# Litianyu141/Gen-FVGN-steady

Hardware: AMD Instinct MI355X
Metric: training iters/sec, 50k-cell cylinder mesh (fwd + loss + bwd + Adam, batch resident in HBM) (higher is better)
Workload: dtype f32

## Files before the change

gen-fvgn-steady_amd/csrc/slice.hip:

```cpp
#include <cstdlib>
#include "gfv_common.h"
#include "gfv_prof.h"
#include "../../include/gfv.h"

namespace {

constexpr int H = 8, D = 16, G = 32;

__global__ __launch_bounds__(256) void slice_softmax_fwd_kernel(const float* __restrict__ xmid, const float* __restrict__ Ws,
                                                                const float* __restrict__ bs, const float* __restrict__ temp,
                                                                float* __restrict__ w, int N) {
  __shared__ float sW[G * D];
  __shared__ float sB[G];
  __shared__ __attribute__((aligned(16))) float stage[256 * (G + 4)];
  const int tid = threadIdx.x;
  for (int i = tid; i < G * D; i += 256) sW[i] = Ws[i];
  if (tid < G) sB[tid] = bs[tid];
  __syncthreads();
  const long row0 = (long)blockIdx.x * 256;
  const long row = row0 + tid;
  const long nrows = (long)N * H;
  if (row < nrows) {
    const int h = (int)(row & (H - 1));
    float x[D];
// ... 304 lines not shown
    for (int c = 0; c < D; ++c) {
      const float t = sTok[g][c];
      q += t * sWq[j * D + c]; k += t * sWk[j * D + c]; v += t * sWv[j * D + c];
    }
    sQ[g][j] = q; sK[g][j] = k; sV[g][j] = v;
  }
  __syncthreads();
  for (int idx = tid; idx < G * D; idx += 256) {
    const int j = idx / D, c = idx % D;
    float s = 0.f;
    for (int i = 0; i < G; ++i) s += sA[i][j] * sGO[i][c];
    sGV[j][c] = s;
  }
  for (int idx = tid; idx < G * G; idx += 256) {
    const int i = idx / G, j = idx % G;
    float s = 0.f;
#pragma unroll
    for (int c = 0; c < D; ++c) s += sGO[i][c] * sV[j][c];
    sGA[i][j] = s;
  }
  __syncthreads();
  if (tid < G) {
    float dot = 0.f;
    for (int j = 0; j < G; ++j) dot += sA[tid][j] * sGA[tid][j];
    for (int j = 0; j < G; ++j) sGA[tid][j] = sA[tid][j] * (sGA[tid][j] - dot) * A.scale;
  }
  __syncthreads();
  for (int idx = tid; idx < G * D; idx += 256) {
    const int i = idx / D, c = idx % D;
    float gq = 0.f, gk = 0.f;
    for (int j = 0; j < G; ++j) {
      gq += sGA[i][j] * sK[j][c];
      gk += sGA[j][i] * sQ[j][c];
    }
    sGQ[i][c] = gq; sGK[i][c] = gk;
  }
  __syncthreads();
  for (int idx = tid; idx < G * D; idx += 256) {
    const int g = idx / D, c = idx % D;
    float s = 0.f;
#pragma unroll
    for (int j = 0; j < D; ++j) s += sGQ[g][j] * sWq[j * D + c] + sGK[g][j] * sWk[j * D + c] + sGV[g][j] * sWv[j * D + c];
    sGT[g][c] = s;
  }
  {
    const int j = tid / D, c = tid % D;
    float dq = 0.f, dk = 0.f, dv = 0.f;
    for (int g = 0; g < G; ++g) {
      const float t = sTok[g][c];
      dq += sGQ[g][j] * t; dk += sGK[g][j] * t; dv += sGV[g][j] * t;
    }
    float* o = A.dW_partial + (size_t)bh * 3 * D * D;
    o[tid] = dq; o[D * D + tid] = dk; o[2 * D * D + tid] = dv;
  }
  __syncthreads();
  for (int idx = tid; idx < G * D; idx += 256) {
    const int g = idx / D, c = idx % D;
    A.g_raw[(size_t)bh * G * D + idx] = sGT[g][c] / (A.norm[bh * G + g] + 1e-5f);
  }
  if (tid < G) {
    float s = 0.f;
#pragma unroll
    for (int c = 0; c < D; ++c) s += sGT[tid][c] * sTok[tid][c];
    A.g_norm[bh * G + tid] = -s / (A.norm[bh * G + tid] + 1e-5f);
  }
}

constexpr int TS = G * D + 4;

__device__ __forceinline__ bool stage_T(const float* __restrict__ T, const int* __restrict__ batch, int N, float* sT) {
  const int n_first = blockIdx.x * 32;
  const int n_last = min(n_first + 31, N - 1);
  const int b0 = batch[n_first];
  const bool uniform = (batch[n_last] == b0);
  if (uniform) {
    const float4* src = reinterpret_cast<const float4*>(T + (size_t)b0 * H * G * D);
    for (int i = threadIdx.x; i < H * G * D / 4; i += 256) {
      const int h = i / (G * D / 4), r = i % (G * D / 4);
      *reinterpret_cast<float4*>(&sT[h * TS + 4 * r]) = src[i];
    }
  }
  __syncthreads();
  return uniform;
}

__device__ __forceinline__ void deslice_row(const float4* __restrict__ wp, const float* __restrict__ Tp, float (&acc)[D]) {
#pragma unroll
  for (int i = 0; i < 8; ++i) {
    const float4 wv = wp[i];
    const float ww[4] = {wv.x, wv.y, wv.z, wv.w};
#pragma unroll
    for (int k = 0; k < 4; ++k) {
      const float4* tp = reinterpret_cast<const float4*>(Tp + (4 * i + k) * D);
#pragma unroll
      for (int j = 0; j < 4; ++j) {
        const float4 t = tp[j];
        acc[4 * j] += ww[k] * t.x; acc[4 * j + 1] += ww[k] * t.y; acc[4 * j + 2] += ww[k] * t.z; acc[4 * j + 3] += ww[k] * t.w;
      }
    }
  }
}

__global__ __launch_bounds__(256) void deslice_kernel(const float* __restrict__ w, const float* __restrict__ T,
                                                      const int* __restrict__ batch, float* __restrict__ out, int N,
                                                      int accumulate) {
  __shared__ __attribute__((aligned(16))) float sT[H * TS];
  if (accumulate & 2) {
    const int n_first = blockIdx.x * 32;
    if (batch[min(n_first + 31, N - 1)] == batch[n_first]) return;
    accumulate = 0;
  }
  const bool uniform = stage_T(T, batch, N, sT);
  const long row = (long)blockIdx.x * 256 + threadIdx.x;
  if (row >= (long)N * H) return;
  const int n = (int)(row >> 3), h = (int)(row & 7);
  float acc[D];
#pragma unroll
  for (int c = 0; c < D; ++c) acc[c] = 0.f;
  const float4* wp = reinterpret_cast<const float4*>(w + row * G);
  if (uniform) deslice_row(wp, &sT[h * TS], acc);
  else deslice_row(wp, T + ((size_t)batch[n] * H + h) * G * D, acc);
  float4* op = reinterpret_cast<float4*>(out + row * D);
#pragma unroll
  for (int j = 0; j < 4; ++j) {
    float4 v = make_float4(acc[4 * j], acc[4 * j + 1], acc[4 * j + 2], acc[4 * j + 3]);
    if (accumulate) { const float4 p = op[j]; v.x += p.x; v.y += p.y; v.z += p.z; v.w += p.w; }
    op[j] = v;
  }
}

__global__ __launch_bounds__(256) void slice_gw_kernel(const float* __restrict__ a, const float* __restrict__ T,
                                                       const float* __restrict__ add, const int* __restrict__ batch,
                                                       float* __restrict__ gw, int N, int accumulate) {
  __shared__ __attribute__((aligned(16))) float sT[H * TS];
  constexpr int SS = G + 4;
  __shared__ __attribute__((aligned(16))) float stage[256 * SS];
  const bool uniform = stage_T(T, batch, N, sT);
  const int tid = threadIdx.x;
  const long row0 = (long)blockIdx.x * 256;
  const long row = row0 + tid;
  const long nrows = (long)N * H;
  if (row < nrows) {
    const int n = (int)(row >> 3), h = (int)(row & 7);
    const size_t bh = (size_t)batch[n] * H + h;
    float x[D];
    const float4* ap = reinterpret_cast<const float4*>(a + row * D);
#pragma unroll
    for (int i = 0; i < 4; ++i) {
      const float4 v = ap[i];
      x[4 * i] = v.x; x[4 * i + 1] = v.y; x[4 * i + 2] = v.z; x[4 * i + 3] = v.w;
    }
    float4 av[G / 4];
#pragma unroll
    for (int i = 0; i < G / 4; ++i)
      av[i] = add ? reinterpret_cast<const float4*>(add + bh * G)[i] : make_float4(0.f, 0.f, 0.f, 0.f);
    const float* Tp = uniform ? &sT[h * TS] : T + bh * G * D;
#pragma unroll
    for (int i = 0; i < G / 4; ++i) {
      float r[4] = {av[i].x, av[i].y, av[i].z, av[i].w};
#pragma unroll
      for (int k = 0; k < 4; ++k) {
        const float4* tp = reinterpret_cast<const float4*>(Tp + (4 * i + k) * D);
#pragma unroll
        for (int j = 0; j < 4; ++j) {
          const float4 t = tp[j];
          r[k] += x[4 * j] * t.x + x[4 * j + 1] * t.y + x[4 * j + 2] * t.z + x[4 * j + 3] * t.w;
// ... 100 lines not shown
          const float4 t = t2[j];
          r2[k] += fx[4 * j] * t.x + fx[4 * j + 1] * t.y + fx[4 * j + 2] * t.z + fx[4 * j + 3] * t.w;
          acc[4 * j] += wg * t.x; acc[4 * j + 1] += wg * t.y; acc[4 * j + 2] += wg * t.z; acc[4 * j + 3] += wg * t.w;
        }
        gv[4 * i + k] = r2[k] + r1[k];
      }
      __builtin_amdgcn_sched_barrier(0);
    }
    float4* op = reinterpret_cast<float4*>(A.gfxmid + row * D);
#pragma unroll
    for (int j = 0; j < 4; ++j) op[j] = make_float4(acc[4 * j], acc[4 * j + 1], acc[4 * j + 2], acc[4 * j + 3]);
  }
  __syncthreads();
  if (live) {
    float x[D];
    const float4* xp = reinterpret_cast<const float4*>(A.xmid + row * D);
#pragma unroll
    for (int i = 0; i < 4; ++i) {
      const float4 v = xp[i];
      x[4 * i] = v.x; x[4 * i + 1] = v.y; x[4 * i + 2] = v.z; x[4 * i + 3] = v.w;
    }
    float dot = 0.f;
#pragma unroll
    for (int i = 0; i < 8; ++i)
      dot += wv[4 * i] * gv[4 * i] + wv[4 * i + 1] * gv[4 * i + 1] + wv[4 * i + 2] * gv[4 * i + 2] + wv[4 * i + 3] * gv[4 * i + 3];
    float gx[D];
#pragma unroll
    for (int c = 0; c < D; ++c) gx[c] = 0.f;
#pragma unroll
    for (int g = 0; g < G; ++g) {
      const float gz = wv[g] * (gv[g] - dot);
      float lg = 0.f;
#pragma unroll
      for (int c = 0; c < D; ++c) lg += x[c] * sW[g * D + c];
      lg += sB[g];
      dT -= gz * lg * invT * invT;
      const float gl = gz * invT;
      sGL[tid * (G + 1) + g] = gl;
#pragma unroll
      for (int c = 0; c < D; ++c) gx[c] += gl * sW[g * D + c];
    }
    float4* op = reinterpret_cast<float4*>(A.gxmid + row * D);
#pragma unroll
    for (int i = 0; i < 4; ++i) op[i] = make_float4(gx[4 * i], gx[4 * i + 1], gx[4 * i + 2], gx[4 * i + 3]);
#pragma unroll
    for (int c = 0; c < D; ++c) sX[tid * (D + 1) + c] = x[c];
  } else {
#pragma unroll
    for (int g = 0; g < G; ++g) sGL[tid * (G + 1) + g] = 0.f;
#pragma unroll
    for (int c = 0; c < D; ++c) sX[tid * (D + 1) + c] = 0.f;
  }
  __syncthreads();
  sDT[tid] = dT;
  __syncthreads();
  float* out = A.partial + (size_t)blockIdx.x * 552;
  {
    const int wave = tid >> 6, lane = tid & 63, li = lane & 15, kq = lane >> 4;
    if (wave < 2) {
      floatx4 acc = {0.f, 0.f, 0.f, 0.f};
#pragma unroll 8
      for (int ks = 0; ks < 64; ++ks) {
        const int r = 4 * ks + kq;
        const float a = sGL[r * (G + 1) + 16 * wave + li];
        const float b = sX[r * (D + 1) + li];
        acc = __builtin_amdgcn_mfma_f32_16x16x4f32(a, b, acc, 0, 0, 0);
      }
#pragma unroll
      for (int reg = 0; reg < 4; ++reg) out[(16 * wave + 4 * kq + reg) * D + li] = acc[reg];
    }
  }
  if (tid < G) {
    float s = 0.f;
    for (int r = 0; r < 256; ++r) s += sGL[r * (G + 1) + tid];
    out[512 + tid] = s;
  }
  if (tid < H) {
    float s = 0.f;
    for (int r = tid; r < 256; r += H) s += sDT[r];
    out[544 + tid] = s;
  }
}

__global__ __launch_bounds__(256, 2) void slice_post_bwd_mfma_kernel(const SlicePostArgs A) {
  __shared__ __attribute__((aligned(16))) float sT1[H * TS];
  __shared__ __attribute__((aligned(16))) float sT2[H * TS];
  __shared__ __attribute__((aligned(16))) float sWs[G * D];
  __shared__ float sBs[G];
  constexpr int TRS = G + 4;
  __shared__ __attribute__((aligned(16))) float sTr[4][16 * TRS];
  __shared__ float sRed[4][552];
  const int tid = threadIdx.x, wave = tid >> 6, lane = tid & 63, li = lane & 15, q = lane >> 4;
  const int n_first = blockIdx.x * 32;
  const int n_last = min(n_first + 31, A.N - 1);
  const int b0 = A.batch[n_first];
  if (A.batch[n_last] != b0) return;
  {
    const float4* s1 = reinterpret_cast<const float4*>(A.T1 + (size_t)b0 * H * G * D);
    const float4* s2 = reinterpret_cast<const float4*>(A.T2 + (size_t)b0 * H * G * D);
    for (int i = tid; i < H * G * D / 4; i += 256) {
      const int h = i / (G * D / 4), r = i % (G * D / 4);
      *reinterpret_cast<float4*>(&sT1[h * TS + 4 * r]) = s1[i];
      *reinterpret_cast<float4*>(&sT2[h * TS + 4 * r]) = s2[i];
    }
    for (int i = tid; i < G * D; i += 256) sWs[i] = A.Ws[i];
    if (tid < G) sBs[tid] = A.bs[tid];
  }
  __syncthreads();
  float bws[2][4], wsd[2][4], bsv[2];
#pragma unroll
  for (int t = 0; t < 2; ++t) {
    const float4 v = *reinterpret_cast<const float4*>(&sWs[(16 * t + li) * D + 4 * q]);
    bws[t][0] = v.x; bws[t][1] = v.y; bws[t][2] = v.z; bws[t][3] = v.w;
    bsv[t] = sBs[16 * t + li];
#pragma unroll
    for (int s = 0; s < 4; ++s) wsd[t][s] = sWs[(16 * t + 4 * q + s) * D + li];
  }
  floatx4 dws[2] = {{0.f, 0.f, 0.f, 0.f}, {0.f, 0.f, 0.f, 0.f}};
  float dbs[2] = {0.f, 0.f}, dTw[2] = {0.f, 0.f};
  float* tr = sTr[wave];
#pragma unroll 1
  for (int hh = 0; hh < 2; ++hh) {
    const int h = 2 * wave + hh;
    const float invT = 1.0f / A.temp[h];
    float b1[2][4], b2[2][4], t2d[2][4], gnv[2];
#pragma unroll
    for (int t = 0; t < 2; ++t) {
      const float4 u1 = *reinterpret_cast<const float4*>(&sT1[h * TS + (16 * t + li) * D + 4 * q]);
      const float4 u2 = *reinterpret_cast<const float4*>(&sT2[h * TS + (16 * t + li) * D + 4 * q]);
      b1[t][0] = u1.x; b1[t][1] = u1.y; b1[t][2] = u1.z; b1[t][3] = u1.w;
      b2[t][0] = u2.x; b2[t][1] = u2.y; b2[t][2] = u2.z; b2[t][3] = u2.w;
      gnv[t] = A.gnorm[((size_t)b0 * H + h) * G + 16 * t + li];
#pragma unroll
      for (int s = 0; s < 4; ++s) t2d[t][s] = sT2[h * TS + (16 * t + 4 * q + s) * D + li];
    }
#pragma unroll 1
    for (int nt = 0; nt < 2; ++nt) {
      const int n0 = n_first + 16 * nt;
      const int nodeA = n0 + li;
      const bool liveA = nodeA < A.N;
      const size_t rowA = (size_t)(liveA ? nodeA : A.N - 1) * H + h;
      const float mA = liveA ? 1.0f : 0.0f;
      float4 vgo = *reinterpret_cast<const float4*>(A.gox + rowA * D + 4 * q);
      float4 vfx = *reinterpret_cast<const float4*>(A.fxm + rowA * D + 4 * q);
      float4 vx = *reinterpret_cast<const float4*>(A.xmid + rowA * D + 4 * q);
      float4 vw0 = *reinterpret_cast<const float4*>(A.w + rowA * G + 4 * q);
      float4 vw1 = *reinterpret_cast<const float4*>(A.w + rowA * G + 16 + 4 * q);
      const float ago[4] = {vgo.x * mA, vgo.y * mA, vgo.z * mA, vgo.w * mA};
      const float afx[4] = {vfx.x * mA, vfx.y * mA, vfx.z * mA, vfx.w * mA};
      const float ax[4] = {vx.x * mA, vx.y * mA, vx.z * mA, vx.w * mA};
      const float aw[2][4] = {{vw0.x * mA, vw0.y * mA, vw0.z * mA, vw0.w * mA}, {vw1.x * mA, vw1.y * mA, vw1.z * mA, vw1.w * mA}};
      float wd[2][4], xb[4];
      size_t rowD[4];
      bool liveD[4];
#pragma unroll
      for (int r = 0; r < 4; ++r) {
        const int nd = n0 + 4 * q + r;
        liveD[r] = nd < A.N;
        rowD[r] = (size_t)(liveD[r] ? nd : A.N - 1) * H + h;
        const float m = liveD[r] ? 1.0f : 0.0f;
        wd[0][r] = A.w[rowD[r] * G + li] * m;
        wd[1][r] = A.w[rowD[r] * G + 16 + li] * m;
        xb[r] = A.xmid[rowD[r] * D + li] * m;
      }
      floatx4 g2[2], g1[2], lg[2];
#pragma unroll
      for (int t = 0; t < 2; ++t) {
        g2[t] = floatx4{gnv[t], gnv[t], gnv[t], gnv[t]};
        g1[t] = floatx4{0.f, 0.f, 0.f, 0.f};
        lg[t] = floatx4{bsv[t], bsv[t], bsv[t], bsv[t]};
#pragma unroll
        for (int s = 0; s < 4; ++s) {
          g2[t] = __builtin_amdgcn_mfma_f32_16x16x4f32(afx[s], b2[t][s], g2[t], 0, 0, 0);
          g1[t] = __builtin_amdgcn_mfma_f32_16x16x4f32(ago[s], b1[t][s], g1[t], 0, 0, 0);
          lg[t] = __builtin_amdgcn_mfma_f32_16x16x4f32(ax[s], bws[t][s], lg[t], 0, 0, 0);
        }
      }
      float gl[2][4];
#pragma unroll
      for (int r = 0; r < 4; ++r) {
        const float gw0 = g2[0][r] + g1[0][r], gw1 = g2[1][r] + g1[1][r];
        const float dot = gfv_row16_sum(wd[0][r] * gw0 + wd[1][r] * gw1);
        const float gz0 = wd[0][r] * (gw0 - dot), gz1 = wd[1][r] * (gw1 - dot);
        dTw[hh] -= (gz0 * lg[0][r] + gz1 * lg[1][r]) * invT * invT;
        gl[0][r] = gz0 * invT;
        gl[1][r] = gz1 * invT;
      }
#pragma unroll
      for (int t = 0; t < 2; ++t) {
#pragma unroll
        for (int s = 0; s < 4; ++s) dws[t] = __builtin_amdgcn_mfma_f32_16x16x4f32(gl[t][s], xb[s], dws[t], 0, 0, 0);
        dbs[t] += (gl[t][0] + gl[t][1]) + (gl[t][2] + gl[t][3]);
#pragma unroll
        for (int r = 0; r < 4; ++r) tr[(4 * q + r) * TRS + 16 * t + li] = gl[t][r];
      }
      __builtin_amdgcn_wave_barrier();
      floatx4 gxa = {0.f, 0.f, 0.f, 0.f}, gfa = {0.f, 0.f, 0.f, 0.f};
#pragma unroll
      for (int u = 0; u < 2; ++u) {
        const float4 v = *reinterpret_cast<const float4*>(&tr[li * TRS + 16 * u + 4 * q]);
        const float agl[4] = {v.x, v.y, v.z, v.w};
#pragma unroll
        for (int s = 0; s < 4; ++s) {
          gxa = __builtin_amdgcn_mfma_f32_16x16x4f32(agl[s], wsd[u][s], gxa, 0, 0, 0);
          gfa = __builtin_amdgcn_mfma_f32_16x16x4f32(aw[u][s], t2d[u][s], gfa, 0, 0, 0);
        }
      }
      __builtin_amdgcn_wave_barrier();
#pragma unroll
      for (int r = 0; r < 4; ++r) {
        if (liveD[r]) {
          A.gxmid[rowD[r] * D + li] = gxa[r];
          A.gfxmid[rowD[r] * D + li] = gfa[r];
        }
      }
    }
  }
  float* red = sRed[wave];
#pragma unroll
  for (int t = 0; t < 2; ++t) {
#pragma unroll
    for (int r = 0; r < 4; ++r) red[(16 * t + 4 * q + r) * D + li] = dws[t][r];
    float a, b;
    gfv_lane_xor16(dbs[t], a, b);
    const float v = a + b;
    gfv_lane_xor32(v, a, b);
    if (q == 0) red[512 + 16 * t + li] = a + b;
  }
#pragma unroll
  for (int hh = 0; hh < 2; ++hh) {
    const float v = gfv_wave_sum(dTw[hh]);
    if (lane == 0) red[544 + hh] = v;
  }
  __syncthreads();
  float* out = A.partial + (size_t)blockIdx.x * 552;
  for (int i = tid; i < 544; i += 256) out[i] = (sRed[0][i] + sRed[1][i]) + (sRed[2][i] + sRed[3][i]);
  if (tid < H) out[544 + tid] = sRed[tid >> 1][544 + (tid & 1)];
}

template <bool SOFTMAX>
__global__ __launch_bounds__(256, 2) void slice_token_mfma_kernel(const float* __restrict__ xmid, const float* __restrict__ Ws,
                                                                  const float* __restrict__ bs, const float* __restrict__ temp,
                                                                  float* __restrict__ w, const float* __restrict__ a,
                                                                  const int* __restrict__ chunk_beg, const int* __restrict__ chunk_end,
                                                                  float* __restrict__ partial) {
  const int tid = threadIdx.x, wave = tid >> 6, lane = tid & 63, li = lane & 15, q = lane >> 4;
  const int beg = chunk_beg[blockIdx.x], end = chunk_end[blockIdx.x];
  float bws[2][4], bsv[2];
  if (SOFTMAX) {
#pragma unroll
    for (int t = 0; t < 2; ++t) {
      const float4 v = *reinterpret_cast<const float4*>(Ws + (16 * t + li) * D + 4 * q);
      bws[t][0] = v.x; bws[t][1] = v.y; bws[t][2] = v.z; bws[t][3] = v.w;
      bsv[t] = bs[16 * t + li];
    }
  }
  float* out = partial + (size_t)blockIdx.x * 256 * 17;
#pragma unroll 1
  for (int hh = 0; hh < 2; ++hh) {
    const int h = 2 * wave + hh;
    const float invT = SOFTMAX ? 1.0f / temp[h] : 0.f;
    floatx4 tok[2] = {{0.f, 0.f, 0.f, 0.f}, {0.f, 0.f, 0.f, 0.f}};
    float nrm[2] = {0.f, 0.f};
#pragma unroll 1
    for (int n0 = beg; n0 < end; n0 += 16) {
      float wd[2][4], ab[4];
      size_t rowD[4];
      bool liveD[4];
#pragma unroll
      for (int r = 0; r < 4; ++r) {
        const int nd = n0 + 4 * q + r;
        liveD[r] = nd < end;
        rowD[r] = (size_t)(liveD[r] ? nd : end - 1) * H + h;
        ab[r] = liveD[r] ? a[rowD[r] * D + li] : 0.f;
      }
      if (SOFTMAX) {
        const int nA = n0 + li;
        const bool liveA = nA < end;
        const size_t rowA = (size_t)(liveA ? nA : end - 1) * H + h;
        const float4 vx = *reinterpret_cast<const float4*>(xmid + rowA * D + 4 * q);
        const float ax[4] = {vx.x, vx.y, vx.z, vx.w};
        floatx4 lg[2];
#pragma unroll
        for (int t = 0; t < 2; ++t) {
          lg[t] = floatx4{bsv[t], bsv[t], bsv[t], bsv[t]};
#pragma unroll
          for (int s = 0; s < 4; ++s) lg[t] = __builtin_amdgcn_mfma_f32_16x16x4f32(ax[s], bws[t][s], lg[t], 0, 0, 0);
        }
#pragma unroll
        for (int r = 0; r < 4; ++r) {
          const float z0 = lg[0][r] * invT, z1 = lg[1][r] * invT;
          const float mx = gfv_row16_max(fmaxf(z0, z1));
          const float e0 = __expf(z0 - mx), e1 = __expf(z1 - mx);
          const float inv = 1.0f / gfv_row16_sum(e0 + e1);
          const float m = liveD[r] ? 1.0f : 0.0f;
          wd[0][r] = e0 * inv * m;
          wd[1][r] = e1 * inv * m;
          if (liveD[r]) {
            w[rowD[r] * G + li] = wd[0][r];
            w[rowD[r] * G + 16 + li] = wd[1][r];
          }
        }
      } else {
#pragma unroll
        for (int r = 0; r < 4; ++r) {
          wd[0][r] = liveD[r] ? w[rowD[r] * G + li] : 0.f;
          wd[1][r] = liveD[r] ? w[rowD[r] * G + 16 + li] : 0.f;
        }
      }
#pragma unroll
      for (int t = 0; t < 2; ++t) {
#pragma unroll
        for (int s = 0; s < 4; ++s) tok[t] = __builtin_amdgcn_mfma_f32_16x16x4f32(wd[t][s], ab[s], tok[t], 0, 0, 0);
        nrm[t] += (wd[t][0] + wd[t][1]) + (wd[t][2] + wd[t][3]);
      }
    }
#pragma unroll
    for (int t = 0; t < 2; ++t) {
#pragma unroll
      for (int r = 0; r < 4; ++r) out[(size_t)(h * G + 16 * t + 4 * q + r) * 17 + li] = tok[t][r];
      float x0, x1;
      gfv_lane_xor16(nrm[t], x0, x1);
      const float v = x0 + x1;
      gfv_lane_xor32(v, x0, x1);
      if (q == 0) out[(size_t)(h * G + 16 * t + li) * 17 + 16] = x0 + x1;
    }
  }
}

__global__ __launch_bounds__(256, 2) void deslice_mfma_kernel(const float* __restrict__ w, const float* __restrict__ T,
                                                              const int* __restrict__ batch, float* __restrict__ out, int N) {
  const int tid = threadIdx.x, wave = tid >> 6, lane = tid & 63, li = lane & 15, q = lane >> 4;
  const int n_first = blockIdx.x * 32;
  const int n_last = min(n_first + 31, N - 1);
  const int b0 = batch[n_first];
  if (batch[n_last] != b0) return;
#pragma unroll 1
  for (int hh = 0; hh < 2; ++hh) {
    const int h = 2 * wave + hh;
    const float* Tp = T + ((size_t)b0 * H + h) * G * D;
    float t2d[2][4];
#pragma unroll
    for (int u = 0; u < 2; ++u)
#pragma unroll
      for (int s = 0; s < 4; ++s) t2d[u][s] = Tp[(16 * u + 4 * q + s) * D + li];
#pragma unroll
    for (int nt = 0; nt < 2; ++nt) {
      const int nA = n_first + 16 * nt + li;
      const bool liveA = nA < N;
      const size_t rowA = (size_t)(liveA ? nA : N - 1) * H + h;
      const float4 v0 = *reinterpret_cast<const float4*>(w + rowA * G + 4 * q);
      const float4 v1 = *reinterpret_cast<const float4*>(w + rowA * G + 16 + 4 * q);
      const float aw[2][4] = {{v0.x, v0.y, v0.z, v0.w}, {v1.x, v1.y, v1.z, v1.w}};
      floatx4 acc = {0.f, 0.f, 0.f, 0.f};
#pragma unroll
      for (int u = 0; u < 2; ++u)
#pragma unroll
        for (int s = 0; s < 4; ++s) acc = __builtin_amdgcn_mfma_f32_16x16x4f32(aw[u][s], t2d[u][s], acc, 0, 0, 0);
#pragma unroll
      for (int r = 0; r < 4; ++r) {
        const int nd = n_first + 16 * nt + 4 * q + r;
        if (nd < N) out[((size_t)nd * H + h) * D + li] = acc[r];
      }
    }
  }
}

}

extern "C" int gfv_slice_softmax_fwd(const float* xmid, const float* Ws, const float* bs, const float* temp, float* w,
                                     int32_t N, void* stream) {
  GfvProfScope ps_(GFV_K_SLICE, 0, 1536.0 * N, stream);
  if (N <= 0) return N == 0 ? GFV_OK : GFV_ERR_ARG;
  GFV_LAUNCH(slice_softmax_fwd_kernel, dim3(gfv_div_up((long)N * H, 256)), dim3(256), 0, (hipStream_t)stream,
                     xmid, Ws, bs, temp, w, N);
  GFV_CHECK_LAUNCH();
  return GFV_OK;
}

extern "C" int gfv_slice_softmax_bwd_blocks(int32_t N) { return gfv_div_up((long)N * H, 256); }

extern "C" int gfv_slice_softmax_bwd(const float* xmid, const float* Ws, const float* bs, const float* temp,
                                     const float* w, const float* gw, float* gxmid, float* partial, int32_t N,
                                     void* stream) {
  GfvProfScope ps_(GFV_K_SLICE, 0, 3072.0 * N, stream);
  if (N <= 0) return N == 0 ? GFV_OK : GFV_ERR_ARG;
  GFV_LAUNCH(slice_softmax_bwd_kernel, dim3(gfv_div_up((long)N * H, 256)), dim3(256), 0, (hipStream_t)stream,
                     xmid, Ws, bs, temp, w, gw, gxmid, partial, N);
  GFV_CHECK_LAUNCH();
  return GFV_OK;
}

static int slice_mfma_on() {
  static const int on = [] { const char* e = getenv("GFV_SLICE_MFMA"); return e ? atoi(e) : 1; }();
  return on;
}

extern "C" int gfv_slice_token_partial(const float* w, const float* a, const int32_t* chunk_beg, const int32_t* chunk_end,
                                       int32_t n_chunks, float* partial, void* stream) {
  GfvProfScope ps_(GFV_K_SLICE, 0, 64.0 * 1536.0 * n_chunks, stream);
  if (n_chunks <= 0) return n_chunks == 0 ? GFV_OK : GFV_ERR_ARG;
  if (slice_mfma_on())
    GFV_LAUNCH((slice_token_mfma_kernel<false>), dim3(n_chunks), dim3(256), 0, (hipStream_t)stream, nullptr, nullptr, nullptr,
                       nullptr, const_cast<float*>(w), a, chunk_beg, chunk_end, partial);
  else
    GFV_LAUNCH(slice_token_partial_kernel, dim3(n_chunks), dim3(256), 0, (hipStream_t)stream, w, a, chunk_beg,
                       chunk_end, partial);
  GFV_CHECK_LAUNCH();
  return GFV_OK;
}

extern "C" int gfv_slice_softmax_token(const float* xmid, const float* Ws, const float* bs, const float* temp, const float* a,
                                       const int32_t* chunk_beg, const int32_t* chunk_end, int32_t n_chunks, float* w,
                                       float* partial, void* stream) {
  GfvProfScope ps_(GFV_K_SLICE, 0, 64.0 * 2048.0 * n_chunks, stream);
  if (n_chunks <= 0) return n_chunks == 0 ? GFV_OK : GFV_ERR_ARG;
  GFV_LAUNCH((slice_token_mfma_kernel<true>), dim3(n_chunks), dim3(256), 0, (hipStream_t)stream, xmid, Ws, bs, temp, w, a,
                     chunk_beg, chunk_end, partial);
  GFV_CHECK_LAUNCH();
  return GFV_OK;
}

extern "C" int gfv_hidden_size(void);
static float attn_scale() { return 1.0f / sqrtf((float)(gfv_hidden_size() / 8)); }

extern "C" int gfv_slice_attention_fwd(const float* partial, const int32_t* gchunk_ptr, int32_t B, const float* Wq,
                                       const float* Wk, const float* Wv, float* token, float* norm, float* attn,
                                       float* out_token, void* stream) {
  GfvProfScope ps_(GFV_K_SLICE, 0, 60000.0 * B, stream);
  if (B <= 0) return B == 0 ? GFV_OK : GFV_ERR_ARG;
  AttnFwdArgs a{partial, gchunk_ptr, Wq, Wk, Wv, token, norm, attn, out_token, attn_scale()};
  GFV_LAUNCH(slice_attention_fwd_kernel, dim3(B, H), dim3(256), 0, (hipStream_t)stream, a);
  GFV_CHECK_LAUNCH();
  return GFV_OK;
}

extern "C" int gfv_slice_attention_bwd(const float* gpartial, const int32_t* gchunk_ptr, int32_t B, const float* Wq,
                                       const float* Wk, const float* Wv, const float* token, const float* norm,
                                       const float* attn, float* g_raw, float* g_norm, float* dW_partial, void* stream) {
  GfvProfScope ps_(GFV_K_SLICE, 0, 100000.0 * B, stream);
  if (B <= 0) return B == 0 ? GFV_OK : GFV_ERR_ARG;
  AttnBwdArgs a{gpartial, gchunk_ptr, Wq, Wk, Wv, token, norm, attn, g_raw, g_norm, dW_partial, attn_scale()};
  GFV_LAUNCH(slice_attention_bwd_kernel, dim3(B, H), dim3(256), 0, (hipStream_t)stream, a);
  GFV_CHECK_LAUNCH();
  return GFV_OK;
}

extern "C" int gfv_deslice(const float* w, const float* T, const int32_t* batch, float* out, int32_t N, int32_t accumulate,
                           void* stream) {
  GfvProfScope ps_(GFV_K_SLICE, 0, 1536.0 * N, stream);
  if (N <= 0) return N == 0 ? GFV_OK : GFV_ERR_ARG;
  static const int dmfma = [] { const char* e = getenv("GFV_DESLICE_MFMA"); return e ? atoi(e) : 1; }();
  if (dmfma && slice_mfma_on() && !(accumulate & 1)) {
    GFV_LAUNCH(deslice_mfma_kernel, dim3(gfv_div_up((long)N * H, 256)), dim3(256), 0, (hipStream_t)stream, w, T, batch, out, N);
    if (!(accumulate & 4))
      GFV_LAUNCH(deslice_kernel, dim3(gfv_div_up((long)N * H, 256)), dim3(256), 0, (hipStream_t)stream, w, T, batch, out, N, 2);
  } else {
    accumulate &= 1;
    GFV_LAUNCH(deslice_kernel, dim3(gfv_div_up((long)N * H, 256)), dim3(256), 0, (hipStream_t)stream, w, T, batch,
                       out, N, accumulate);
  }
  GFV_CHECK_LAUNCH();
  return GFV_OK;
}

extern "C" int gfv_slice_gw(const float* a, const float* T, const float* add, const int32_t* batch, float* gw, int32_t N,
                            int32_t accumulate, void* stream) {
  GfvProfScope ps_(GFV_K_SLICE, 0, (accumulate ? 3072.0 : 1536.0) * N, stream);
  if (N <= 0) return N == 0 ? GFV_OK : GFV_ERR_ARG;
  GFV_LAUNCH(slice_gw_kernel, dim3(gfv_div_up((long)N * H, 256)), dim3(256), 0, (hipStream_t)stream, a, T, add,
                     batch, gw, N, accumulate);
  GFV_CHECK_LAUNCH();
  return GFV_OK;
}

extern "C" int gfv_slice_post_bwd(const float* xmid, const float* Ws, const float* bs, const float* temp, const float* w,
                                  const float* g_out_x, const float* out_token, const float* fx_mid, const float* g_raw,
                                  const float* g_norm, const int32_t* batch, float* g_x_mid, float* g_fx_mid, float* partial,
                                  int32_t N, int32_t n_graphs, void* stream) {
  GfvProfScope ps_(GFV_K_SLICE, 0, (3 * 512.0 + 1024.0 + 2 * 512.0) * N, stream);
  if (N <= 0) return N == 0 ? GFV_OK : GFV_ERR_ARG;
  SlicePostArgs a{xmid, Ws, bs, temp, w, g_out_x, out_token, fx_mid, g_raw, g_norm, batch, g_x_mid, g_fx_mid, partial, N, 0};
  static const int mfma = [] { const char* e = getenv("GFV_SLICE_MFMA"); return e ? atoi(e) : 1; }();
  const dim3 grid(gfv_div_up((long)N * H, 256));
  if (mfma) {
    GFV_LAUNCH(slice_post_bwd_mfma_kernel, grid, dim3(256), 0, (hipStream_t)stream, a);
    if (n_graphs != 1) {
      a.only_straddling = 1;
      GFV_LAUNCH(slice_post_bwd_kernel, grid, dim3(256), 0, (hipStream_t)stream, a);
    }
  } else {
    GFV_LAUNCH(slice_post_bwd_kernel, grid, dim3(256), 0, (hipStream_t)stream, a);
  }
  GFV_CHECK_LAUNCH();
  return GFV_OK;
}
```

Measured before the change: 285.6.

## Use one wave per head in slice MFMA kernels with staged coalesced outputs

The slice post-backward and token MFMA kernels grow from 256 to 512 threads, so each of the 8 heads gets its own wave instead of each wave looping over two heads. The post-backward kernel issues its global loads before the batch-uniformity check and builds the transposed operands through a per-wave LDS transpose instead of strided global reads. It also stages gradient outputs in LDS for coalesced float4 row stores, and chains the weight-gradient MFMA accumulation across wave pairs. The token kernel batches 64 nodes of loads ahead of compute behind a sched barrier. The aim is more parallelism and memory-level overlap, at the cost of more registers and LDS per block, fewer resident blocks, and an extra block-wide sync.

```diff
diff --git a/gen-fvgn-steady_amd/csrc/slice.hip b/gen-fvgn-steady_amd/csrc/slice.hip
--- a/gen-fvgn-steady_amd/csrc/slice.hip
+++ b/gen-fvgn-steady_amd/csrc/slice.hip
@@ -410,6 +410,15 @@
   }
   __syncthreads();
   return uniform;
+}
+
+__device__ __forceinline__ void store_rows32(const float* sOut, float* __restrict__ out, int n_first, int N) {
+  for (int i = threadIdx.x; i < 32 * (H * D / 4); i += blockDim.x) {
+    const int row = i >> 5, c4 = i & 31;
+    if (n_first + row < N)
+      reinterpret_cast<float4*>(out + (size_t)(n_first + row) * (H * D))[c4] =
+          *reinterpret_cast<const float4*>(&sOut[row * (H * D) + 4 * c4]);
+  }
 }
 
 __device__ __forceinline__ void deslice_row(const float4* __restrict__ wp, const float* __restrict__ Tp, float (&acc)[D]) {
@@ -676,169 +685,217 @@
   }
 }
 
-__global__ __launch_bounds__(256, 2) void slice_post_bwd_mfma_kernel(const SlicePostArgs A) {
-  __shared__ __attribute__((aligned(16))) float sT1[H * TS];
-  __shared__ __attribute__((aligned(16))) float sT2[H * TS];
+__device__ __forceinline__ void post_bwd_chain(const float (&glk)[2][2][4], const float (&xbk)[2][4], floatx4 (&dws)[2], float (&dbs)[2]) {
+#pragma unroll
+  for (int nt = 0; nt < 2; ++nt)
+#pragma unroll
+    for (int t = 0; t < 2; ++t) {
+#pragma unroll
+      for (int s = 0; s < 4; ++s) dws[t] = __builtin_amdgcn_mfma_f32_16x16x4f32(glk[nt][t][s], xbk[nt][s], dws[t], 0, 0, 0);
+      dbs[t] += (glk[nt][t][0] + glk[nt][t][1]) + (glk[nt][t][2] + glk[nt][t][3]);
+    }
+}
+
+constexpr int POST_THREADS = 64 * H;
+__global__ __launch_bounds__(POST_THREADS) void slice_post_bwd_mfma_kernel(const SlicePostArgs A) {
+  __shared__ __attribute__((aligned(16))) float sT[2 * H * TS];
+  static_assert(2 * 32 * H * D <= 2 * H * TS, "the two output tiles fit the region of the slice tensors");
+  float* sT1 = sT;
+  float* sT2 = sT + H * TS;
   __shared__ __attribute__((aligned(16))) float sWs[G * D];
   __shared__ float sBs[G];
-  constexpr int TRS = G + 4;
-  __shared__ __attribute__((aligned(16))) float sTr[4][16 * TRS];
-  __shared__ float sRed[4][552];
+  constexpr int TRS = G + D + 4;
+  __shared__ __attribute__((aligned(16))) float sTr[H][16 * TRS];
+  __shared__ float sRed[4][544];
+  __shared__ float sDT[H];
   const int tid = threadIdx.x, wave = tid >> 6, lane = tid & 63, li = lane & 15, q = lane >> 4;
+  const int h = wave;
   const int n_first = blockIdx.x * 32;
   const int n_last = min(n_first + 31, A.N - 1);
+  float4 vgo[2], vfx[2], vx[2], vw0[2], vw1[2];
+#pragma unroll
+  for (int nt = 0; nt < 2; ++nt) {
+    const int nodeA = n_first + 16 * nt + li;
+    const size_t rowA = (size_t)(nodeA < A.N ? nodeA : A.N - 1) * H + h;
+    vgo[nt] = *reinterpret_cast<const float4*>(A.gox + rowA * D + 4 * q);
+    vfx[nt] = *reinterpret_cast<const float4*>(A.fxm + rowA * D + 4 * q);
+    vx[nt] = *reinterpret_cast<const float4*>(A.xmid + rowA * D + 4 * q);
+    vw0[nt] = *reinterpret_cast<const float4*>(A.w + rowA * G + 4 * q);
+    vw1[nt] = *reinterpret_cast<const float4*>(A.w + rowA * G + 16 + 4 * q);
+  }
   const int b0 = A.batch[n_first];
   if (A.batch[n_last] != b0) return;
+  const float invT = 1.0f / A.temp[h];
+  float gnv[2];
+#pragma unroll
+  for (int t = 0; t < 2; ++t) gnv[t] = A.gnorm[((size_t)b0 * H + h) * G + 16 * t + li];
   {
     const float4* s1 = reinterpret_cast<const float4*>(A.T1 + (size_t)b0 * H * G * D);
     const float4* s2 = reinterpret_cast<const float4*>(A.T2 + (size_t)b0 * H * G * D);
-    for (int i = tid; i < H * G * D / 4; i += 256) {
-      const int h = i / (G * D / 4), r = i % (G * D / 4);
-      *reinterpret_cast<float4*>(&sT1[h * TS + 4 * r]) = s1[i];
-      *reinterpret_cast<float4*>(&sT2[h * TS + 4 * r]) = s2[i];
-    }
-    for (int i = tid; i < G * D; i += 256) sWs[i] = A.Ws[i];
-    if (tid < G) sBs[tid] = A.bs[tid];
-  }
-  __syncthreads();
-  float bws[2][4], wsd[2][4], bsv[2];
+    float4 u1[2], u2[2];
+#pragma unroll
+    for (int k = 0; k < 2; ++k) {
+      u1[k] = s1[tid + POST_THREADS * k];
+      u2[k] = s2[tid + POST_THREADS * k];
+    }
+    const float ws0 = A.Ws[tid];
+    const float bsl = A.bs[tid & (G - 1)];
+#pragma unroll
+    for (int k = 0; k < 2; ++k) {
+      const int i = tid + POST_THREADS * k, hs = i / (G * D / 4), r = i % (G * D / 4);
+      *reinterpret_cast<float4*>(&sT1[hs * TS + 4 * r]) = u1[k];
+      *reinterpret_cast<float4*>(&sT2[hs * TS + 4 * r]) = u2[k];
+    }
+    sWs[tid] = ws0;
+    if (tid < G) sBs[tid] = bsl;
+  }
+  __syncthreads();
+  float bws[2][4], wsd[2][4], bsv[2], b1[2][4], b2[2][4], t2d[2][4];
 #pragma unroll
   for (int t = 0; t < 2; ++t) {
     const float4 v = *reinterpret_cast<const float4*>(&sWs[(16 * t + li) * D + 4 * q]);
     bws[t][0] = v.x; bws[t][1] = v.y; bws[t][2] = v.z; bws[t][3] = v.w;
     bsv[t] = sBs[16 * t + li];
-#pragma unroll
-    for (int s = 0; s < 4; ++s) wsd[t][s] = sWs[(16 * t + 4 * q + s) * D + li];
-  }
+    const float4 u1 = *reinterpret_cast<const float4*>(&sT1[h * TS + (16 * t + li) * D + 4 * q]);
+    const float4 u2 = *reinterpret_cast<const float4*>(&sT2[h * TS + (16 * t + li) * D + 4 * q]);
+    b1[t][0] = u1.x; b1[t][1] = u1.y; b1[t][2] = u1.z; b1[t][3] = u1.w;
+    b2[t][0] = u2.x; b2[t][1] = u2.y; b2[t][2] = u2.z; b2[t][3] = u2.w;
+#pragma unroll
+    for (int s = 0; s < 4; ++s) {
+      wsd[t][s] = sWs[(16 * t + 4 * q + s) * D + li];
+      t2d[t][s] = sT2[h * TS + (16 * t + 4 * q + s) * D + li];
+    }
+  }
+  float dTw = 0.f;
+  float glk[2][2][4], xbk[2][4];
+  floatx4 gxo[2], gfo[2];
+  float* tr = sTr[wave];
+#pragma unroll
+  for (int nt = 0; nt < 2; ++nt) {
+    const int n0 = n_first + 16 * nt;
+    const float mA = n0 + li < A.N ? 1.0f : 0.0f;
+    const float ago[4] = {vgo[nt].x * mA, vgo[nt].y * mA, vgo[nt].z * mA, vgo[nt].w * mA};
+    const float afx[4] = {vfx[nt].x * mA, vfx[nt].y * mA, vfx[nt].z * mA, vfx[nt].w * mA};
+    const float ax[4] = {vx[nt].x * mA, vx[nt].y * mA, vx[nt].z * mA, vx[nt].w * mA};
+    const float aw[2][4] = {{vw0[nt].x * mA, vw0[nt].y * mA, vw0[nt].z * mA, vw0[nt].w * mA},
+                            {vw1[nt].x * mA, vw1[nt].y * mA, vw1[nt].z * mA, vw1[nt].w * mA}};
+    *reinterpret_cast<float4*>(&tr[li * TRS + 4 * q]) = make_float4(aw[0][0], aw[0][1], aw[0][2], aw[0][3]);
+    *reinterpret_cast<float4*>(&tr[li * TRS + 16 + 4 * q]) = make_float4(aw[1][0], aw[1][1], aw[1][2], aw[1][3]);
+    *reinterpret_cast<float4*>(&tr[li * TRS + G + 4 * q]) = make_float4(ax[0], ax[1], ax[2], ax[3]);
+    __builtin_amdgcn_wave_barrier();
+    float wd[2][4];
+#pragma unroll
+    for (int r = 0; r < 4; ++r) {
+      wd[0][r] = tr[(4 * q + r) * TRS + li];
+      wd[1][r] = tr[(4 * q + r) * TRS + 16 + li];
+      xbk[nt][r] = tr[(4 * q + r) * TRS + G + li];
+    }
+    __builtin_amdgcn_wave_barrier();
+    floatx4 g2[2], g1[2], lg[2];
+#pragma unroll
+    for (int t = 0; t < 2; ++t) {
+      g2[t] = floatx4{gnv[t], gnv[t], gnv[t], gnv[t]};
+      g1[t] = floatx4{0.f, 0.f, 0.f, 0.f};
+      lg[t] = floatx4{bsv[t], bsv[t], bsv[t], bsv[t]};
+#pragma unroll
+      for (int s = 0; s < 4; ++s) {
+        g2[t] = __builtin_amdgcn_mfma_f32_16x16x4f32(afx[s], b2[t][s], g2[t], 0, 0, 0);
+        g1[t] = __builtin_amdgcn_mfma_f32_16x16x4f32(ago[s], b1[t][s], g1[t], 0, 0, 0);
+        lg[t] = __builtin_amdgcn_mfma_f32_16x16x4f32(ax[s], bws[t][s], lg[t], 0, 0, 0);
+      }
+    }
+#pragma unroll
+    for (int r = 0; r < 4; ++r) {
+      const float gw0 = g2[0][r] + g1[0][r], gw1 = g2[1][r] + g1[1][r];
+      const float dot = gfv_row16_sum(wd[0][r] * gw0 + wd[1][r] * gw1);
+      const float gz0 = wd[0][r] * (gw0 - dot), gz1 = wd[1][r] * (gw1 - dot);
+      dTw -= (gz0 * lg[0][r] + gz1 * lg[1][r]) * invT * invT;
+      glk[nt][0][r] = gz0 * invT;
+      glk[nt][1][r] = gz1 * invT;
+    }
+#pragma unroll
+    for (int t = 0; t < 2; ++t)
+#pragma unroll
+      for (int r = 0; r < 4; ++r) tr[(4 * q + r) * TRS + 16 * t + li] = glk[nt][t][r];
+    __builtin_amdgcn_wave_barrier();
+    floatx4 gxa = {0.f, 0.f, 0.f, 0.f}, gfa = {0.f, 0.f, 0.f, 0.f};
+#pragma unroll
+    for (int u = 0; u < 2; ++u) {
+      const float4 v = *reinterpret_cast<const float4*>(&tr[li * TRS + 16 * u + 4 * q]);
+      const float agl[4] = {v.x, v.y, v.z, v.w};
+#pragma unroll
+      for (int s = 0; s < 4; ++s) {
+        gxa = __builtin_amdgcn_mfma_f32_16x16x4f32(agl[s], wsd[u][s], gxa, 0, 0, 0);
+        gfa = __builtin_amdgcn_mfma_f32_16x16x4f32(aw[u][s], t2d[u][s], gfa, 0, 0, 0);
+      }
+    }
+    __builtin_amdgcn_wave_barrier();
+    gxo[nt] = gxa;
+    gfo[nt] = gfa;
+  }
+  float* red = sRed[wave >> 1];
   floatx4 dws[2] = {{0.f, 0.f, 0.f, 0.f}, {0.f, 0.f, 0.f, 0.f}};
-  float dbs[2] = {0.f, 0.f}, dTw[2] = {0.f, 0.f};
-  float* tr = sTr[wave];
-#pragma unroll 1
-  for (int hh = 0; hh < 2; ++hh) {
-    const int h = 2 * wave + hh;
-    const float invT = 1.0f / A.temp[h];
-    float b1[2][4], b2[2][4], t2d[2][4], gnv[2];
+  float dbs[2] = {0.f, 0.f};
+  if (!(wave & 1)) {
+    post_bwd_chain(glk, xbk, dws, dbs);
 #pragma unroll
     for (int t = 0; t < 2; ++t) {
-      const float4 u1 = *reinterpret_cast<const float4*>(&sT1[h * TS + (16 * t + li) * D + 4 * q]);
-      const float4 u2 = *reinterpret_cast<const float4*>(&sT2[h * TS + (16 * t + li) * D + 4 * q]);
-      b1[t][0] = u1.x; b1[t][1] = u1.y; b1[t][2] = u1.z; b1[t][3] = u1.w;
-      b2[t][0] = u2.x; b2[t][1] = u2.y; b2[t][2] = u2.z; b2[t][3] = u2.w;
-      gnv[t] = A.gnorm[((size_t)b0 * H + h) * G + 16 * t + li];
-#pragma unroll
-      for (int s = 0; s < 4; ++s) t2d[t][s] = sT2[h * TS + (16 * t + 4 * q + s) * D + li];
-    }
-#pragma unroll 1
-    for (int nt = 0; nt < 2; ++nt) {
-      const int n0 = n_first + 16 * nt;
-      const int nodeA = n0 + li;
-      const bool liveA = nodeA < A.N;
-      const size_t rowA = (size_t)(liveA ? nodeA : A.N - 1) * H + h;
-      const float mA = liveA ? 1.0f : 0.0f;
-      float4 vgo = *reinterpret_cast<const float4*>(A.gox + rowA * D + 4 * q);
-      float4 vfx = *reinterpret_cast<const float4*>(A.fxm + rowA * D + 4 * q);
-      float4 vx = *reinterpret_cast<const float4*>(A.xmid + rowA * D + 4 * q);
-      float4 vw0 = *reinterpret_cast<const float4*>(A.w + rowA * G + 4 * q);
-      float4 vw1 = *reinterpret_cast<const float4*>(A.w + rowA * G + 16 + 4 * q);
-      const float ago[4] = {vgo.x * mA, vgo.y * mA, vgo.z * mA, vgo.w * mA};
-      const float afx[4] = {vfx.x * mA, vfx.y * mA, vfx.z * mA, vfx.w * mA};
-      const float ax[4] = {vx.x * mA, vx.y * mA, vx.z * mA, vx.w * mA};
-      const float aw[2][4] = {{vw0.x * mA, vw0.y * mA, vw0.z * mA, vw0.w * mA}, {vw1.x * mA, vw1.y * mA, vw1.z * mA, vw1.w * mA}};
-      float wd[2][4], xb[4];
-      size_t rowD[4];
-      bool liveD[4];
-#pragma unroll
-      for (int r = 0; r < 4; ++r) {
-        const int nd = n0 + 4 * q + r;
-        liveD[r] = nd < A.N;
-        rowD[r] = (size_t)(liveD[r] ? nd : A.N - 1) * H + h;
-        const float m = liveD[r] ? 1.0f : 0.0f;
-        wd[0][r] = A.w[rowD[r] * G + li] * m;
-        wd[1][r] = A.w[rowD[r] * G + 16 + li] * m;
-        xb[r] = A.xmid[rowD[r] * D + li] * m;
-      }
-      floatx4 g2[2], g1[2], lg[2];
-#pragma unroll
-      for (int t = 0; t < 2; ++t) {
-        g2[t] = floatx4{gnv[t], gnv[t], gnv[t], gnv[t]};
-        g1[t] = floatx4{0.f, 0.f, 0.f, 0.f};
-        lg[t] = floatx4{bsv[t], bsv[t], bsv[t], bsv[t]};
-#pragma unroll
-        for (int s = 0; s < 4; ++s) {
-          g2[t] = __builtin_amdgcn_mfma_f32_16x16x4f32(afx[s], b2[t][s], g2[t], 0, 0, 0);
-          g1[t] = __builtin_amdgcn_mfma_f32_16x16x4f32(ago[s], b1[t][s], g1[t], 0, 0, 0);
-          lg[t] = __builtin_amdgcn_mfma_f32_16x16x4f32(ax[s], bws[t][s], lg[t], 0, 0, 0);
-        }
-      }
-      float gl[2][4];
-#pragma unroll
-      for (int r = 0; r < 4; ++r) {
-        const float gw0 = g2[0][r] + g1[0][r], gw1 = g2[1][r] + g1[1][r];
-        const float dot = gfv_row16_sum(wd[0][r] * gw0 + wd[1][r] * gw1);
-        const float gz0 = wd[0][r] * (gw0 - dot), gz1 = wd[1][r] * (gw1 - dot);
-        dTw[hh] -= (gz0 * lg[0][r] + gz1 * lg[1][r]) * invT * invT;
-        gl[0][r] = gz0 * invT;
-        gl[1][r] = gz1 * invT;
-      }
-#pragma unroll
-      for (int t = 0; t < 2; ++t) {
-#pragma unroll
-        for (int s = 0; s < 4; ++s) dws[t] = __builtin_amdgcn_mfma_f32_16x16x4f32(gl[t][s], xb[s], dws[t], 0, 0, 0);
-        dbs[t] += (gl[t][0] + gl[t][1]) + (gl[t][2] + gl[t][3]);
-#pragma unroll
-        for (int r = 0; r < 4; ++r) tr[(4 * q + r) * TRS + 16 * t + li] = gl[t][r];
-      }
-      __builtin_amdgcn_wave_barrier();
-      floatx4 gxa = {0.f, 0.f, 0.f, 0.f}, gfa = {0.f, 0.f, 0.f, 0.f};
-#pragma unroll
-      for (int u = 0; u < 2; ++u) {
-        const float4 v = *reinterpret_cast<const float4*>(&tr[li * TRS + 16 * u + 4 * q]);
-        const float agl[4] = {v.x, v.y, v.z, v.w};
-#pragma unroll
-        for (int s = 0; s < 4; ++s) {
-          gxa = __builtin_amdgcn_mfma_f32_16x16x4f32(agl[s], wsd[u][s], gxa, 0, 0, 0);
-          gfa = __builtin_amdgcn_mfma_f32_16x16x4f32(aw[u][s], t2d[u][s], gfa, 0, 0, 0);
-        }
-      }
-      __builtin_amdgcn_wave_barrier();
-#pragma unroll
-      for (int r = 0; r < 4; ++r) {
-        if (liveD[r]) {
-          A.gxmid[rowD[r] * D + li] = gxa[r];
-          A.gfxmid[rowD[r] * D + li] = gfa[r];
-        }
-      }
-    }
-  }
-  float* red = sRed[wave];
-#pragma unroll
-  for (int t = 0; t < 2; ++t) {
-#pragma unroll
-    for (int r = 0; r < 4; ++r) red[(16 * t + 4 * q + r) * D + li] = dws[t][r];
-    float a, b;
-    gfv_lane_xor16(dbs[t], a, b);
-    const float v = a + b;
-    gfv_lane_xor32(v, a, b);
-    if (q == 0) red[512 + 16 * t + li] = a + b;
-  }
-#pragma unroll
-  for (int hh = 0; hh < 2; ++hh) {
-    const float v = gfv_wave_sum(dTw[hh]);
-    if (lane == 0) red[544 + hh] = v;
-  }
+#pragma unroll
+      for (int r = 0; r < 4; ++r) red[(16 * t + 4 * q + r) * D + li] = dws[t][r];
+      tr[16 * t * 4 + lane] = dbs[t];
+    }
+  }
+  __syncthreads();
+  if (wave & 1) {
+    const float* tre = sTr[wave - 1];
+#pragma unroll
+    for (int t = 0; t < 2; ++t) {
+#pragma unroll
+      for (int r = 0; r < 4; ++r) dws[t][r] = red[(16 * t + 4 * q + r) * D + li];
+      dbs[t] = tre[16 * t * 4 + lane];
+    }
+    post_bwd_chain(glk, xbk, dws, dbs);
+#pragma unroll
+    for (int t = 0; t < 2; ++t) {
+#pragma unroll
+      for (int r = 0; r < 4; ++r) red[(16 * t + 4 * q + r) * D + li] = dws[t][r];
+      float a, b;
+      gfv_lane_xor16(dbs[t], a, b);
+      const float v = a + b;
+      gfv_lane_xor32(v, a, b);
+      if (q == 0) red[512 + 16 * t + li] = a + b;
+    }
+  }
+  {
+    const float v = gfv_wave_sum(dTw);
+    if (lane == 0) sDT[h] = v;
+  }
+  float* sGx = sT;
+  float* sGf = sT + 32 * H * D;
+#pragma unroll
+  for (int nt = 0; nt < 2; ++nt)
+#pragma unroll
+    for (int r = 0; r < 4; ++r) {
+      const int row = 16 * nt + 4 * q + r;
+      sGx[row * (H * D) + h * D + li] = gxo[nt][r];
+      sGf[row * (H * D) + h * D + li] = gfo[nt][r];
+    }
   __syncthreads();
   float* out = A.partial + (size_t)blockIdx.x * 552;
-  for (int i = tid; i < 544; i += 256) out[i] = (sRed[0][i] + sRed[1][i]) + (sRed[2][i] + sRed[3][i]);
-  if (tid < H) out[544 + tid] = sRed[tid >> 1][544 + (tid & 1)];
-}
-
+  for (int i = tid; i < 544; i += POST_THREADS) out[i] = (sRed[0][i] + sRed[1][i]) + (sRed[2][i] + sRed[3][i]);
+  if (tid < H) out[544 + tid] = sDT[tid];
+  store_rows32(sGx, A.gxmid, n_first, A.N);
+  store_rows32(sGf, A.gfxmid, n_first, A.N);
+}
+
+constexpr int TOK_THREADS = 64 * H;
 template <bool SOFTMAX>
-__global__ __launch_bounds__(256, 2) void slice_token_mfma_kernel(const float* __restrict__ xmid, const float* __restrict__ Ws,
+__global__ __launch_bounds__(TOK_THREADS) void slice_token_mfma_kernel(const float* __restrict__ xmid, const float* __restrict__ Ws,
                                                                   const float* __restrict__ bs, const float* __restrict__ temp,
                                                                   float* __restrict__ w, const float* __restrict__ a,
                                                                   const int* __restrict__ chunk_beg, const int* __restrict__ chunk_end,
                                                                   float* __restrict__ partial) {
-  const int tid = threadIdx.x, wave = tid >> 6, lane = tid & 63, li = lane & 15, q = lane >> 4;
+  const int tid = threadIdx.x, h = tid >> 6, lane = tid & 63, li = lane & 15, q = lane >> 4;
   const int beg = chunk_beg[blockIdx.x], end = chunk_end[blockIdx.x];
   float bws[2][4], bsv[2];
   if (SOFTMAX) {
@@ -849,76 +906,93 @@
       bsv[t] = bs[16 * t + li];
     }
   }
+  const float invT = SOFTMAX ? 1.0f / temp[h] : 0.f;
   float* out = partial + (size_t)blockIdx.x * 256 * 17;
+  floatx4 tok[2] = {{0.f, 0.f, 0.f, 0.f}, {0.f, 0.f, 0.f, 0.f}};
+  float nrm[2] = {0.f, 0.f};
 #pragma unroll 1
-  for (int hh = 0; hh < 2; ++hh) {
-    const int h = 2 * wave + hh;
-    const float invT = SOFTMAX ? 1.0f / temp[h] : 0.f;
-    floatx4 tok[2] = {{0.f, 0.f, 0.f, 0.f}, {0.f, 0.f, 0.f, 0.f}};
-    float nrm[2] = {0.f, 0.f};
-#pragma unroll 1
-    for (int n0 = beg; n0 < end; n0 += 16) {
-      float wd[2][4], ab[4];
-      size_t rowD[4];
-      bool liveD[4];
+  for (int base = beg; base < end; base += 64) {
+    float ab[4][4], wl[4][2][4];
+    float4 vx[4];
+#pragma unroll
+    for (int nt = 0; nt < 4; ++nt) {
+      const int n0 = base + 16 * nt;
 #pragma unroll
       for (int r = 0; r < 4; ++r) {
         const int nd = n0 + 4 * q + r;
-        liveD[r] = nd < end;
-        rowD[r] = (size_t)(liveD[r] ? nd : end - 1) * H + h;
-        ab[r] = liveD[r] ? a[rowD[r] * D + li] : 0.f;
+        const size_t row = (size_t)(nd < end ? nd : end - 1) * H + h;
+        ab[nt][r] = a[row * D + li];
+        if (!SOFTMAX) {
+          wl[nt][0][r] = w[row * G + li];
+          wl[nt][1][r] = w[row * G + 16 + li];
+        }
       }
       if (SOFTMAX) {
         const int nA = n0 + li;
-        const bool liveA = nA < end;
-        const size_t rowA = (size_t)(liveA ? nA : end - 1) * H + h;
-        const float4 vx = *reinterpret_cast<const float4*>(xmid + rowA * D + 4 * q);
-        const float ax[4] = {vx.x, vx.y, vx.z, vx.w};
-        floatx4 lg[2];
-#pragma unroll
-        for (int t = 0; t < 2; ++t) {
-          lg[t] = floatx4{bsv[t], bsv[t], bsv[t], bsv[t]};
-#pragma unroll
-          for (int s = 0; s < 4; ++s) lg[t] = __builtin_amdgcn_mfma_f32_16x16x4f32(ax[s], bws[t][s], lg[t], 0, 0, 0);
-        }
-#pragma unroll
-        for (int r = 0; r < 4; ++r) {
-          const float z0 = lg[0][r] * invT, z1 = lg[1][r] * invT;
-          const float mx = gfv_row16_max(fmaxf(z0, z1));
-          const float e0 = __expf(z0 - mx), e1 = __expf(z1 - mx);
-          const float inv = 1.0f / gfv_row16_sum(e0 + e1);
-          const float m = liveD[r] ? 1.0f : 0.0f;
-          wd[0][r] = e0 * inv * m;
-          wd[1][r] = e1 * inv * m;
-          if (liveD[r]) {
-            w[rowD[r] * G + li] = wd[0][r];
-            w[rowD[r] * G + 16 + li] = wd[1][r];
+        const size_t rowA = (size_t)(nA < end ? nA : end - 1) * H + h;
+        vx[nt] = *reinterpret_cast<const float4*>(xmid + rowA * D + 4 * q);
+      }
+    }
+    __builtin_amdgcn_sched_barrier(0);
+#pragma unroll
+    for (int nt = 0; nt < 4; ++nt) {
+      const int n0 = base + 16 * nt;
+      {
+        float wd[2][4], am[4];
+#pragma unroll
+        for (int r = 0; r < 4; ++r) am[r] = n0 + 4 * q + r < end ? ab[nt][r] : 0.f;
+        if (SOFTMAX) {
+          const float ax[4] = {vx[nt].x, vx[nt].y, vx[nt].z, vx[nt].w};
+          floatx4 lg[2];
+#pragma unroll
+          for (int t = 0; t < 2; ++t) {
+            lg[t] = floatx4{bsv[t], bsv[t], bsv[t], bsv[t]};
+#pragma unroll
+            for (int s = 0; s < 4; ++s) lg[t] = __builtin_amdgcn_mfma_f32_16x16x4f32(ax[s], bws[t][s], lg[t], 0, 0, 0);
+          }
+#pragma unroll
+          for (int r = 0; r < 4; ++r) {
+            const int nd = n0 + 4 * q + r;
+            const bool live = nd < end;
+            const float z0 = lg[0][r] * invT, z1 = lg[1][r] * invT;
+            const float mx = gfv_row16_max(fmaxf(z0, z1));
+            const float e0 = __expf(z0 - mx), e1 = __expf(z1 - mx);
+            const float inv = 1.0f / gfv_row16_sum(e0 + e1);
+            const float m = live ? 1.0f : 0.0f;
+            wd[0][r] = e0 * inv * m;
+            wd[1][r] = e1 * inv * m;
+            if (live) {
+              const size_t row = (size_t)nd * H + h;
+              w[row * G + li] = wd[0][r];
+              w[row * G + 16 + li] = wd[1][r];
+            }
+          }
+        } else {
+#pragma unroll
+          for (int r = 0; r < 4; ++r) {
+            const bool live = n0 + 4 * q + r < end;
+            wd[0][r] = live ? wl[nt][0][r] : 0.f;
+            wd[1][r] = live ? wl[nt][1][r] : 0.f;
           }
         }
-      } else {
-#pragma unroll
-        for (int r = 0; r < 4; ++r) {
-          wd[0][r] = liveD[r] ? w[rowD[r] * G + li] : 0.f;
-          wd[1][r] = liveD[r] ? w[rowD[r] * G + 16 + li] : 0.f;
+#pragma unroll
+        for (int t = 0; t < 2; ++t) {
+#pragma unroll
+          for (int s = 0; s < 4; ++s) tok[t] = __builtin_amdgcn_mfma_f32_16x16x4f32(wd[t][s], am[s], tok[t], 0, 0, 0);
+          nrm[t] += (wd[t][0] + wd[t][1]) + (wd[t][2] + wd[t][3]);
         }
       }
-#pragma unroll
-      for (int t = 0; t < 2; ++t) {
-#pragma unroll
-        for (int s = 0; s < 4; ++s) tok[t] = __builtin_amdgcn_mfma_f32_16x16x4f32(wd[t][s], ab[s], tok[t], 0, 0, 0);
-        nrm[t] += (wd[t][0] + wd[t][1]) + (wd[t][2] + wd[t][3]);
-      }
-    }
-#pragma unroll
-    for (int t = 0; t < 2; ++t) {
-#pragma unroll
-      for (int r = 0; r < 4; ++r) out[(size_t)(h * G + 16 * t + 4 * q + r) * 17 + li] = tok[t][r];
-      float x0, x1;
-      gfv_lane_xor16(nrm[t], x0, x1);
-      const float v = x0 + x1;
-      gfv_lane_xor32(v, x0, x1);
-      if (q == 0) out[(size_t)(h * G + 16 * t + li) * 17 + 16] = x0 + x1;
-    }
+    }
+  }
+#pragma unroll
+  for (int t = 0; t < 2; ++t) {
+#pragma unroll
+    for (int r = 0; r < 4; ++r) out[(size_t)(h * G + 16 * t + 4 * q + r) * 17 + li] = tok[t][r];
+    float x0, x1;
+    gfv_lane_xor16(nrm[t], x0, x1);
+    const float v = x0 + x1;
+    gfv_lane_xor32(v, x0, x1);
+    if (q == 0) out[(size_t)(h * G + 16 * t + li) * 17 + 16] = x0 + x1;
   }
 }
 
@@ -995,7 +1069,7 @@
   GfvProfScope ps_(GFV_K_SLICE, 0, 64.0 * 1536.0 * n_chunks, stream);
   if (n_chunks <= 0) return n_chunks == 0 ? GFV_OK : GFV_ERR_ARG;
   if (slice_mfma_on())
-    GFV_LAUNCH((slice_token_mfma_kernel<false>), dim3(n_chunks), dim3(256), 0, (hipStream_t)stream, nullptr, nullptr, nullptr,
+    GFV_LAUNCH((slice_token_mfma_kernel<false>), dim3(n_chunks), dim3(TOK_THREADS), 0, (hipStream_t)stream, nullptr, nullptr, nullptr,
                        nullptr, const_cast<float*>(w), a, chunk_beg, chunk_end, partial);
   else
     GFV_LAUNCH(slice_token_partial_kernel, dim3(n_chunks), dim3(256), 0, (hipStream_t)stream, w, a, chunk_beg,
@@ -1009,7 +1083,7 @@
                                        float* partial, void* stream) {
   GfvProfScope ps_(GFV_K_SLICE, 0, 64.0 * 2048.0 * n_chunks, stream);
   if (n_chunks <= 0) return n_chunks == 0 ? GFV_OK : GFV_ERR_ARG;
-  GFV_LAUNCH((slice_token_mfma_kernel<true>), dim3(n_chunks), dim3(256), 0, (hipStream_t)stream, xmid, Ws, bs, temp, w, a,
+  GFV_LAUNCH((slice_token_mfma_kernel<true>), dim3(n_chunks), dim3(TOK_THREADS), 0, (hipStream_t)stream, xmid, Ws, bs, temp, w, a,
                      chunk_beg, chunk_end, partial);
   GFV_CHECK_LAUNCH();
   return GFV_OK;
@@ -1078,7 +1152,7 @@
   static const int mfma = [] { const char* e = getenv("GFV_SLICE_MFMA"); return e ? atoi(e) : 1; }();
   const dim3 grid(gfv_div_up((long)N * H, 256));
   if (mfma) {
-    GFV_LAUNCH(slice_post_bwd_mfma_kernel, grid, dim3(256), 0, (hipStream_t)stream, a);
+    GFV_LAUNCH(slice_post_bwd_mfma_kernel, grid, dim3(POST_THREADS), 0, (hipStream_t)stream, a);
     if (n_graphs != 1) {
       a.only_straddling = 1;
       GFV_LAUNCH(slice_post_bwd_kernel, grid, dim3(256), 0, (hipStream_t)stream, a);
```

After: 288.2, median of 6. No clear change (+0.9%).
